# doing-science-to-stuff/ndt

Hardware: AMD Instinct MI355X
Metric: Mray/s (primary+shadow+reflect) at 1920x1080 (higher is better)
Workload: dtype f64

## Files before the change

ndt_amd/csrc/ndt_api.hip:

```cpp
#include "ndt_ctx.hpp"
#include <ctype.h>


static thread_local char g_err[512] = "";
int ndt_impl::fail(int code, const char *fmt, ...)
{
    va_list ap;
    va_start(ap, fmt);
    vsnprintf(g_err, sizeof(g_err), fmt, ap);
    va_end(ap);
    return code;
}

extern "C" const char *ndt_hip_last_error(void) { return g_err; }
extern "C" int ndt_hip_abi_version(void) { return NDT_HIP_ABI_VERSION; }

extern "C" int32_t ndt_hip_shard_rows(int32_t height, int32_t row_begin, int32_t row_step)
{
    if (row_step < 1 || row_begin < 0 || row_begin >= height) return 0;
    return (height - row_begin + row_step - 1) / row_step;
}

static const NdtKernelTable *table_for(int dims)
{
    switch (dims) {
    case 3: return ndt_kernel_table_3();
    case 4: return ndt_kernel_table_4();
    case 5: return ndt_kernel_table_5();
    case 6: return ndt_kernel_table_6();
    case 7: return ndt_kernel_table_7();
    case 8: return ndt_kernel_table_8();
    case 9: return ndt_kernel_table_9();
    case 10: return ndt_kernel_table_10();
    case 11: return ndt_kernel_table_11();
    case 12: return ndt_kernel_table_12();
    default: return nullptr;
    }
}

extern "C" int ndt_hip_create(int device, ndt_hip_ctx **out)
{
    if (!out) return fail(NDT_E_INVALID, "ndt_hip_create: out is NULL");
    *out = nullptr;
    int count = 0;
    hipError_t e = hipGetDeviceCount(&count);
    if (e != hipSuccess || count <= 0)
        return fail(NDT_E_DEVICE, "no HIP device available (%s); libndt_hip has no CPU path",
                    e == hipSuccess ? "device count is 0" : hipGetErrorString(e));
    if (device < 0 || device >= count) return fail(NDT_E_INVALID, "device %d out of range (have %d)", device, count);
    HIP_TRY(hipSetDevice(device));
    hipDeviceProp_t prop;
    HIP_TRY(hipGetDeviceProperties(&prop, device));
    if (strncmp(prop.gcnArchName, "gfx950", 6) != 0)
        return fail(NDT_E_DEVICE, "device %d is %s; this library carries gfx950 code objects only", device, prop.gcnArchName);
    ndt_hip_ctx *ctx = new ndt_hip_ctx();
    ctx->device = device;
    {
        static const char *const names[] = { "hybrid_level", "stream_below", "stream_below_list", "hull_box", "face_box", "face_tree", "face_groups", "item_sets", "gate_prepass", "gate_prepass_below", "item_boxes", "leaf_history", "leaf_scan", "leaf_scan_group", "multi_path", "sample_seed", "stream_fused", "fuse_primaries", "shade_pair", "light_window", "debug_levels",
                                             "exit_probe", "shade_probe", "stream_probe", "test_small_pool" };
        const char *pl = getenv("NDT_HIP_PIPELINE");
        if (pl) (void)ndt_hip_set_option(ctx, "pipeline", !strcmp(pl, "levels") ? 1 : !strcmp(pl, "stream") ? 2 : !strcmp(pl, "hybrid") ? 3 : 0);
        for (const char *nm : names) {
            char env[64] = "NDT_HIP_";
            size_t k = strlen(env);
            for (const char *q = nm; *q && k + 1 < sizeof(env); ++q) env[k++] = (char)toupper((unsigned char)*q);
            env[k] = 0;
            const char *v = getenv(env);
            if (v && *v) (void)ndt_hip_set_option(ctx, nm, !strcmp(nm, "shade_probe") ? atoll(v) + 1 : atoll(v));
        }
        if (getenv("NDT_HIP_NO_HULL_BOX")) ctx->hull_box = false;
        if (getenv("NDT_HIP_NO_FACE_BOX")) ctx->face_box = false;
        if (getenv("NDT_HIP_NO_SHADE_PAIR") && atoi(getenv("NDT_HIP_NO_SHADE_PAIR"))) ctx->shade_pair = false;
    }
    e = hipStreamCreateWithFlags(&ctx->stream, hipStreamNonBlocking);
    if (e != hipSuccess) {
        delete ctx;
        return fail(NDT_E_DEVICE, "hipStreamCreate: %s", hipGetErrorString(e));
    }
    e = hipHostMalloc((void **)&ctx->h_counters, 128 * sizeof(int), hipHostMallocDefault);
    if (e == hipSuccess) e = hipHostMalloc((void **)&ctx->h_levels, (NDT_MAX_LEVELS + 1) * sizeof(LevelRange), hipHostMallocDefault);
    if (e == hipSuccess) e = hipHostMalloc((void **)&ctx->h_mail, (NDT_MAX_LEVELS + 2) * sizeof(LevelRange), hipHostMallocMapped | hipHostMallocCoherent);
    if (e == hipSuccess) e = hipHostMalloc((void **)&ctx->h_mail_tag, (NDT_MAX_LEVELS + 2) * sizeof(unsigned long long), hipHostMallocMapped | hipHostMallocCoherent);
    if (e == hipSuccess) e = hipHostGetDevicePointer((void **)&ctx->d_mail, ctx->h_mail, 0);
    if (e == hipSuccess) e = hipHostGetDevicePointer((void **)&ctx->d_mail_tag, ctx->h_mail_tag, 0);
    if (e == hipSuccess) memset(ctx->h_mail_tag, 0, (NDT_MAX_LEVELS + 2) * sizeof(unsigned long long));
    if (e == hipSuccess) e = hipHostMalloc((void **)&ctx->h_done, 16 * sizeof(unsigned long long), hipHostMallocMapped | hipHostMallocCoherent);
    if (e == hipSuccess) e = hipHostGetDevicePointer((void **)&ctx->d_done, ctx->h_done, 0);
    if (e == hipSuccess) memset(ctx->h_done, 0, 16 * sizeof(unsigned long long));
    if (e != hipSuccess) {
        (void)hipStreamDestroy(ctx->stream);
        delete ctx;
        return fail(NDT_E_DEVICE, "hipHostMalloc: %s", hipGetErrorString(e));
    }
    *out = ctx;
    return NDT_OK;
}

extern "C" int ndt_hip_destroy(ndt_hip_ctx *ctx)
{
    if (!ctx) return NDT_OK;
    worker_stop(ctx);
    (void)hipSetDevice(ctx->device);
    (void)hipStreamSynchronize(ctx->stream);
    free_workspace(ctx);
    free_stage(ctx);
    free_async(ctx);
    if (ctx->d_shard) (void)hipFree(ctx->d_shard);
    if (ctx->d_image) (void)hipFree(ctx->d_image);
    for (auto &slot : ctx->pool)
        if (slot.first) (void)hipFree(slot.first);
    for (auto &slot : ctx->pool2)
        if (slot.first) (void)hipFree(slot.first);
    if (ctx->d_blob) (void)hipFree(ctx->d_blob);
    if (ctx->d_out) (void)hipFree(ctx->d_out);
    if (ctx->d_fit) (void)hipFree(ctx->d_fit);
    free_kd(ctx);
    free_png(ctx);
    free_jpeg(ctx);
    free_depth(ctx);
    free_ssaa(ctx);
    if (ctx->d_eyes) (void)hipFree(ctx->d_eyes);
    if (ctx->h_counters) (void)hipHostFree(ctx->h_counters);
    if (ctx->h_levels) (void)hipHostFree(ctx->h_levels);
    if (ctx->h_mail) (void)hipHostFree(ctx->h_mail);
    if (ctx->h_mail_tag) (void)hipHostFree(ctx->h_mail_tag);
    if (ctx->h_done) (void)hipHostFree(ctx->h_done);
    for (hipEvent_t ev : ctx->ev_pool) (void)hipEventDestroy(ev);
    (void)hipStreamDestroy(ctx->stream);
    delete ctx;
    return NDT_OK;
}

extern "C" int ndt_hip_set_option(ndt_hip_ctx *ctx, const char *name, int64_t value)
{
    if (!ctx || !name) return fail(NDT_E_INVALID, "NULL argument");
    const bool on = value != 0;
    if (!strcmp(name, "pipeline")) {
        if (value < 0 || value > 3) return fail(NDT_E_INVALID, "pipeline %lld", (long long)value);
        ctx->pipeline = (int)value;
    } else if (!strcmp(name, "hybrid_level")) ctx->hybrid_level = (int)value;
    else if (!strcmp(name, "stream_below")) ctx->stream_below = value;
    else if (!strcmp(name, "stream_below_list")) ctx->stream_below_list = value;
    else if (!strcmp(name, "hull_box")) ctx->hull_box = on;
    else if (!strcmp(name, "face_box")) ctx->face_box = on;
    else if (!strcmp(name, "face_tree")) ctx->face_tree = on;
    else if (!strcmp(name, "face_groups")) ctx->face_groups = on;
    else if (!strcmp(name, "item_sets")) ctx->item_sets = on;
    else if (!strcmp(name, "item_boxes")) ctx->item_boxes = on;
    else if (!strcmp(name, "gate_prepass_below")) ctx->gate_prepass_below = value;
    else if (!strcmp(name, "gate_prepass")) ctx->gate_prepass = value < 0 ? 0 : value > 2 ? 2 : (int)value;
    else if (!strcmp(name, "sample_seed")) ctx->sample_seed = value;
    else if (!strcmp(name, "leaf_scan")) ctx->leaf_scan = on;
    else if (!strcmp(name, "leaf_scan_group")) ctx->leaf_scan_group = value < 1 ? 1 : value > 64 ? 64 : (int)value;
    else if (!strcmp(name, "leaf_history")) ctx->leaf_history = value < 0 ? 0 : value > 4 ? 4 : (int)value;
    else if (!strcmp(name, "multi_path")) {
        if (value < 0 || value > 2) return fail(NDT_E_INVALID, "multi_path %lld", (long long)value);
        ctx->multi_path = (int)value;
    } else if (!strcmp(name, "stream_fused")) ctx->stream_fused = on;
    else if (!strcmp(name, "fuse_primaries")) ctx->fuse_primaries = value < 0 ? -1 : on ? 1 : 0;
    else if (!strcmp(name, "shade_pair")) ctx->shade_pair = on;
    else if (!strcmp(name, "light_window")) {
        if (value < 0 || value > 64) return fail(NDT_E_INVALID, "light_window %lld (0 auto, 1 .. 64)", (long long)value);
        ctx->light_window = (int)value;
        if (ctx->have_scene) light_windows(ctx);
    }
    else if (!strcmp(name, "debug_levels")) ctx->debug_levels = on;
    else if (!strcmp(name, "exit_probe")) ctx->exit_probe = on;
    else if (!strcmp(name, "shade_probe")) ctx->shade_probe = (int)value - 1;
    else if (!strcmp(name, "stream_probe")) ctx->stream_probe = on;
    else if (!strcmp(name, "test_small_pool")) ctx->test_small_pool = on;
    else return fail(NDT_E_INVALID, "unknown option '%s'", name);
    return NDT_OK;
}

extern "C" void *ndt_hip_stream(ndt_hip_ctx *ctx) { return ctx ? (void *)ctx->stream : nullptr; }
extern "C" int ndt_hip_synchronize(ndt_hip_ctx *ctx)
{
    if (!ctx) return fail(NDT_E_INVALID, "ctx is NULL");
    HIP_TRY(hipSetDevice(ctx->device));
    HIP_TRY(hipStreamSynchronize(ctx->stream));
    return NDT_OK;
}

extern "C" int ndt_hip_upload_scene(ndt_hip_ctx *ctx, const ndt_flat_scene *fs)
{
    if (!ctx || !fs) return fail(NDT_E_INVALID, "NULL argument");
    if (fs->abi_version != NDT_HIP_ABI_VERSION) return fail(NDT_E_INVALID, "scene ABI %d, library ABI %d", fs->abi_version, NDT_HIP_ABI_VERSION);
    if (fs->dims < NDT_MIN_DIMS || fs->dims > NDT_MAX_DIMS)
        return fail(NDT_E_UNSUPPORTED, "%d dimensions: kernels are built for %d..%d", fs->dims, NDT_MIN_DIMS, NDT_MAX_DIMS);
    if (fs->cam_type < 0 || fs->cam_type > 2) return fail(NDT_E_UNSUPPORTED, "camera type %d", fs->cam_type);
    if (fs->cam_type != 0 && (fs->cam_local_x_off < 0 || fs->cam_local_y_off < 0 || fs->cam_local_z_off < 0))
        return fail(NDT_E_INVALID, "VR / panorama cameras need the local axes (camera.h:69-71) in the flat scene");
    if (fs->n_lights < 0 || fs->n_lights > NDT_MAX_LIGHTS) return fail(NDT_E_UNSUPPORTED, "%d lights (max %d)", fs->n_lights, NDT_MAX_LIGHTS);
    if (fs->n_objects < 0 || fs->n_items < 0 || fs->n_items > fs->n_objects) return fail(NDT_E_INVALID, "object counts");
    if (fs->n_kd_nodes < 0 || fs->n_inf < 0 || fs->n_leaf_refs < 0) return fail(NDT_E_INVALID, "kd-tree counts");
    if (fs->n_objects > 0 && !fs->objects) return fail(NDT_E_INVALID, "objects is NULL");
    if (fs->n_lights > 0 && !fs->lights) return fail(NDT_E_INVALID, "lights is NULL");
    if (!fs->vecs) return fail(NDT_E_INVALID, "vecs is NULL");
    HIP_TRY(hipSetDevice(ctx->device));
    ctx->have_scene = false;
    int rc = build_blob(ctx, fs);
    if (rc) return rc;
    ctx->dims = fs->dims;
    ctx->kt = table_for(fs->dims);
    if (!ctx->kt) return fail(NDT_E_UNSUPPORTED, "no kernels for %d dimensions", fs->dims);
    HIP_TRY(hipStreamSynchronize(ctx->stream));
    if (ctx->d_blob_words < ctx->blob.size()) {
        if (ctx->d_blob) HIP_TRY(hipFree(ctx->d_blob));
        ctx->d_blob = nullptr;
        HIP_TRY(hipMalloc((void **)&ctx->d_blob, ctx->blob.size() * sizeof(double)));
        ctx->d_blob_words = ctx->blob.size();
    }
    HIP_TRY(hipMemcpyAsync(ctx->d_blob, ctx->blob.data(), ctx->blob.size() * sizeof(double), hipMemcpyHostToDevice, ctx->stream));
    HIP_TRY(hipStreamSynchronize(ctx->stream));
    ctx->aperture_radius = fs->cam_aperture_radius;
    ctx->have_scene = true;
    if (ctx->debug_levels)
        fprintf(stderr, "ndt_hip: scene blob: %d-D, %d items / %d objects, %d kd nodes of depth %d; %d words staged by the trace kernels (%d KB), %d in all; tier %d, %d mask word(s)\n",
                ctx->dims, ctx->sd.n_items, ctx->sd.n_objects, ctx->sd.n_kd_nodes, ctx->sd.kd_depth, ctx->sd.trace_words, ctx->sd.trace_words / 128,
                ctx->sd.total_words, ctx->tier, ctx->sd.mask_words);
    return NDT_OK;
}

__global__ void k_quantize(const double *rgba, unsigned char *out, long long n_values)
{
    const long long i = (long long)blockIdx.x * blockDim.x + threadIdx.x;
    if (i >= n_values) return;
    const double d = rgba[i];
    double m = (1.0 < d) ? 1.0 : d;
    m = (0.0 > m) ? 0.0 : m;
    out[i] = (unsigned char)(sqrt(m) * 255);
}

extern "C" int ndt_hip_quantize_device(ndt_hip_ctx *ctx, const void *d_rgba, void *d_rgba8, int64_t n_pixels)
{
    if (!ctx || !d_rgba || !d_rgba8 || n_pixels < 0) return fail(NDT_E_INVALID, "bad argument");
    HIP_TRY(hipSetDevice(ctx->device));
    const long long n = n_pixels * 4;
    if (n == 0) return NDT_OK;
// ... 81 lines not shown
```

ndt_amd/csrc/ndt_ctx.hpp:

```cpp
#pragma once
#include <hip/hip_runtime.h>
#include <hip/hip_ext.h>
#include <math.h>
#include <stdarg.h>
#include <stdio.h>
#include <stdlib.h>
#include <string.h>
#include <time.h>
#include <functional>
#include <string>
#include <vector>

#include "../../include/ndt_hip.h"
#include "ndt_kernels.hpp"

namespace ndt_impl {

struct CtxWorker;

int fail(int code, const char *fmt, ...) __attribute__((format(printf, 2, 3)));

}
using namespace ndt_impl;

// ... 20 lines not shown
           info_bytes = 0;
    void *h_info = nullptr;
};

struct JpegState {
    void *d_rgba8 = nullptr, *d_coef = nullptr, *d_slots = nullptr, *d_meta = nullptr, *d_offsets = nullptr, *d_file = nullptr, *d_info = nullptr;
    size_t rgba8_bytes = 0, coef_bytes = 0, slots_bytes = 0, meta_bytes = 0, offsets_bytes = 0, file_bytes = 0, info_bytes = 0;
    void *h_info = nullptr;
};

struct DepthState {
    void *d_records = nullptr;
    void *d_rgba8 = nullptr, *d_depth8 = nullptr;
    size_t records_bytes = 0, rgba8_bytes = 0, depth8_bytes = 0;
    void *h_result = nullptr;
    int launches = 0;
    double finish_ms = 0.0;
};

struct SsaaState {
    void *d_pass = nullptr;
    void *d_acc = nullptr;
    void *d_rgba8 = nullptr, *d_depth8 = nullptr;
    size_t pass_bytes = 0, acc_bytes = 0, rgba8_bytes = 0, depth8_bytes = 0;
    hipEvent_t ev[16] = {};
    int launches = 0;
    int factor = 0;
    double fold_ms = 0.0;
};

struct ndt_hip_ctx {
    int device = 0;
    hipStream_t stream = nullptr;
    const NdtKernelTable *kt = nullptr;
    int dims = 0;
    bool have_scene = false;
    double aperture_radius = 0.0;
    int cam_type = 0;
    bool have_eyes = false, have_local_axes = false;
    bool has_area_lights = false;
    SceneDesc sd{};
    std::vector<double> blob;
    double *d_blob = nullptr;
    size_t d_blob_words = 0;
    int tier = 0;
    int n_shadow_lights = 0;
    struct LightWindow {
        int first, count;
        int n_seg;
        unsigned long long ambient_bits;
    };
    int light_window = 0;
    std::vector<int> light_types;
    std::vector<LightWindow> windows;
    Workspace ws{};
    std::vector<void *> ws_allocs;
    std::vector<void *> sa_allocs;
    std::vector<std::pair<void *, size_t>> pool;
    std::vector<std::pair<void *, size_t>> pool2;
    long long ws_dims = 0;
    long long ws_slab_words = 0;
    int ws_nseg = 0;
    int pipeline = 0;
    int hybrid_level = 2;
    long long stream_below = 1000000;
    long long stream_below_list = 30000;
    StreamArgs sa{};
    bool stream_probe = false, exit_probe = false, debug_levels = false, test_small_pool = false;
    bool hull_box = true, face_box = true, shade_pair = true;
    bool face_tree = true;
    bool face_groups = true;
    int fuse_primaries = -1;
    bool stream_fused = true;
    bool item_sets = true;
    int gate_prepass = 2;
    long long gate_prepass_below = 400000;
    bool item_boxes = true;
    int leaf_scan_group = 64;
    bool leaf_scan = true;
    int leaf_history = 4;
    int shade_probe = -1;
    long long sa_cap = 0, sa_sh_cap = 0;
    int sa_nseg = 0;
    void *d_eyes = nullptr;
    size_t d_eyes_bytes = 0;
    void *d_fit = nullptr;
    size_t d_fit_bytes = 0;
    int fit_launches = 0;
    KdState kd;
    PngState png;
    JpegState jpeg;
    DepthState depth;
    SsaaState ssaa;
    void *d_out = nullptr;
    size_t d_out_bytes = 0;
    void *d_shard = nullptr;
    size_t d_shard_bytes = 0;
    void *d_image = nullptr;
    size_t d_image_bytes = 0;
    void *d_rgba8[2] = { nullptr, nullptr };
    size_t d_rgba8_bytes[2] = { 0, 0 };
    hipStream_t copy_stream = nullptr;
// ... 7 lines not shown
    long long sample_seed = 0;
    int multi_path = 0;
    int multi_path_taken = 0;
    ndt_impl::CtxWorker *worker = nullptr;
    int *h_counters = nullptr;
    LevelRange *h_levels = nullptr;
    LevelRange *h_mail = nullptr;
    unsigned long long *h_mail_tag = nullptr;
    LevelRange *d_mail = nullptr;
    unsigned long long *d_mail_tag = nullptr;
    unsigned long long frame_tag = 0;
    unsigned long long *h_done = nullptr;
    unsigned long long *d_done = nullptr;
    std::vector<hipEvent_t> ev_pool;
};

namespace ndt_impl {

struct HullFaces {
    std::vector<double> rows;
    std::vector<unsigned long long> possible;
    int n_faces = 0;
};
bool hcube_hull_box(const ndt_flat_scene *fs, const ndt_flat_object &o, int n, std::vector<double> &rows, HullFaces *faces = nullptr);
void hcube_face_tree(const HullFaces &hf, int n, std::vector<double> &rows, std::vector<int> &level_off, int &top);
void hcube_face_groups(const HullFaces &hf, const std::vector<double> &hull_rows, int n, std::vector<double> &clusters, std::vector<int> &table,
                       std::vector<int> &face_set, std::vector<int> &members);
bool scene_item_boxes(const ndt_flat_scene *fs, int n, std::vector<double> &frame, std::vector<double> &rows, std::vector<char> &has);
int build_blob(ndt_hip_ctx *ctx, const ndt_flat_scene *fs);
void light_windows(ndt_hip_ctx *ctx);
SceneDesc window_desc(const ndt_hip_ctx *ctx, const SceneDesc &sd, int k);

void free_workspace(ndt_hip_ctx *ctx);
int ensure_workspace(ndt_hip_ctx *ctx, long long cap, long long sh_cap);
int render_pass(ndt_hip_ctx *ctx, RenderGeom rg, bool prof, void *d_rgba, ndt_render_stats &st, void *d_depth = nullptr);
void launch_fill_black(hipStream_t s, double *rgba, long long n_pixels);
void add_stats(ndt_render_stats &acc, const ndt_render_stats &st);

void print_stream_probe(const unsigned int *wave_log, float kernel_ms);
void print_shade_probe(const unsigned int *shade_log, int shade_probe, long long finish_waves);
void print_exit_probe(const unsigned int *exit_log, int launches);
void print_phase_timing(const unsigned long long *dbg);

void worker_stop(ndt_hip_ctx *ctx);
void free_stage(ndt_hip_ctx *ctx);
void free_async(ndt_hip_ctx *ctx);

int fit_spheres_device(ndt_hip_ctx *ctx, int dims, long long n_lists, const int64_t *first, const double *points, const double *point_radius,
                       double *centers, double *radii);

int build_kdtree_device(ndt_hip_ctx *ctx, int dims, int n_items, const double *lower, const double *upper, const unsigned char *finite);
void free_kd(ndt_hip_ctx *ctx);

void free_png(ndt_hip_ctx *ctx);

void free_jpeg(ndt_hip_ctx *ctx);

void free_depth(ndt_hip_ctx *ctx);

void free_ssaa(ndt_hip_ctx *ctx);

int render_antialiased(ndt_hip_ctx *ctx, const ndt_render_params *p, void *d_rgba, ndt_render_stats &total, void *d_depth = nullptr);
void launch_anaglyph(hipStream_t s, const double *left, const double *right, double *out, long long n_pixels);
int render_sampled(ndt_hip_ctx *ctx, const ndt_render_params *p, void *d_rgba, ndt_render_stats &total, void *d_depth = nullptr);
struct SampledList {
    const double *d_pos;
// ... 85 lines not shown
```

ndt_amd/csrc/ndt_frame.hip:

```cpp
#include "ndt_ctx.hpp"
#include "ndt_finish.hpp"
#include <stddef.h>

static void free_stream_args(ndt_hip_ctx *ctx)
{
    for (void *p : ctx->sa_allocs) (void)hipFree(p);
    ctx->sa_allocs.clear();
    memset(&ctx->sa, 0, sizeof(ctx->sa));
    ctx->sa_cap = ctx->sa_sh_cap = 0;
    ctx->sa_nseg = 0;
}

void ndt_impl::free_workspace(ndt_hip_ctx *ctx)
{
    for (void *p : ctx->ws_allocs) (void)hipFree(p);
    ctx->ws_allocs.clear();
    free_stream_args(ctx);
    memset(&ctx->ws, 0, sizeof(ctx->ws));
    ctx->ws_slab_words = 0;
    ctx->ws_dims = 0;
    ctx->ws_nseg = 0;
}


template <typename T> static int ws_alloc(ndt_hip_ctx *ctx, T **p, size_t count, bool stream_args = false)
{
    void *q = nullptr;
    hipError_t e = hipMalloc(&q, (count > 0 ? count : 1) * sizeof(T));
    if (e != hipSuccess) {
        (void)hipGetLastError();
        return fail(NDT_E_NOMEM, "hipMalloc of %zu bytes: %s", count * sizeof(T), hipGetErrorString(e));
    }
    (stream_args ? ctx->sa_allocs : ctx->ws_allocs).push_back(q);
    *p = (T *)q;
    return NDT_OK;
}

int ndt_impl::ensure_workspace(ndt_hip_ctx *ctx, long long cap, long long sh_cap)
{
    Workspace &ws = ctx->ws;
    const bool need_slab = ctx->tier == 1;
    const long long slab_lanes = 2048LL * NDT_TRACE_BLOCK;
    const long long slab_words = need_slab ? slab_lanes * ctx->sd.mask_words : 0;
    if (ws.cap >= cap && ws.sh_cap >= sh_cap && ctx->ws_dims == ctx->dims && ctx->ws_slab_words >= slab_words &&
        ctx->ws_nseg >= ctx->n_shadow_lights)
        return NDT_OK;
    if (cap < ws.cap) cap = ws.cap;
    if (sh_cap < ws.sh_cap) sh_cap = ws.sh_cap;
    cap = (cap + 63) & ~63LL;
    sh_cap = (sh_cap + 63) & ~63LL;
    HIP_TRY(hipStreamSynchronize(ctx->stream));
    free_workspace(ctx);
    const int n = ctx->dims;
    int rc;
    auto give_up = [&](int code) {
        free_workspace(ctx);
        return code;
    };
    ws.cap = cap;
    ws.sh_cap = sh_cap;
    if ((rc = ws_alloc(ctx, &ws.ray_o, (size_t)n * cap))) return give_up(rc);
    if ((rc = ws_alloc(ctx, &ws.ray_v, (size_t)n * cap))) return give_up(rc);
    if ((rc = ws_alloc(ctx, &ws.frac, (size_t)cap))) return give_up(rc);
    if ((rc = ws_alloc(ctx, &ws.depth, (size_t)cap))) return give_up(rc);
    if ((rc = ws_alloc(ctx, &ws.rng_key, (size_t)cap))) return give_up(rc);
    if ((rc = ws_alloc(ctx, &ws.depth_left, (size_t)cap))) return give_up(rc);
    if ((rc = ws_alloc(ctx, &ws.hit_obj, (size_t)cap))) return give_up(rc);
    if ((rc = ws_alloc(ctx, &ws.hit_prim, (size_t)cap))) return give_up(rc);
    if ((rc = ws_alloc(ctx, &ws.hit_p, (size_t)n * cap))) return give_up(rc);
    if ((rc = ws_alloc(ctx, &ws.hit_n, (size_t)n * cap))) return give_up(rc);
    if ((rc = ws_alloc(ctx, &ws.clr, (size_t)3 * cap))) return give_up(rc);
    if ((rc = ws_alloc(ctx, &ws.child_refl, (size_t)cap))) return give_up(rc);
    if ((rc = ws_alloc(ctx, &ws.child_refr, (size_t)cap))) return give_up(rc);
    if ((rc = ws_alloc(ctx, &ws.sh_idx, (size_t)cap * (ctx->n_shadow_lights > 0 ? ctx->n_shadow_lights : 1)))) return give_up(rc);
    if ((rc = ws_alloc(ctx, &ws.sh_mask, (size_t)cap))) return give_up(rc);
    if ((rc = ws_alloc(ctx, &ws.count, (size_t)cap))) return give_up(rc);
    if ((rc = ws_alloc(ctx, &ws.so, (size_t)n * sh_cap))) return give_up(rc);
    if ((rc = ws_alloc(ctx, &ws.sv, (size_t)n * sh_cap))) return give_up(rc);
    if ((rc = ws_alloc(ctx, &ws.slim, (size_t)sh_cap))) return give_up(rc);
    if ((rc = ws_alloc(ctx, &ws.sobj, (size_t)sh_cap))) return give_up(rc);
    if ((rc = ws_alloc(ctx, &ws.sprim, (size_t)sh_cap))) return give_up(rc);
    if ((rc = ws_alloc(ctx, &ws.counters, NDT_CNT_ALLOC))) return give_up(rc);
    if ((rc = ws_alloc(ctx, &ws.ref_rays, 64 * 8))) return give_up(rc);
    if ((rc = ws_alloc(ctx, &ws.dbg, 160))) return give_up(rc);
    if ((rc = ws_alloc(ctx, &ws.exit_log, (size_t)NDT_EXIT_LOG_LAUNCHES * NDT_EXIT_LOG_WORDS))) return give_up(rc);
    if (ctx->shade_probe >= 0 && (rc = ws_alloc(ctx, &ws.shade_log, (size_t)2 * NDT_SHADE_LOG_WAVES))) return give_up(rc);
    if ((rc = ws_alloc(ctx, &ws.levels, NDT_MAX_LEVELS + 1))) return give_up(rc);
    ws.mask_slab_lanes = slab_lanes;
    if (need_slab) {
        if ((rc = ws_alloc(ctx, &ws.mask_slab, (size_t)slab_words))) return give_up(rc);
    }
    ctx->ws_slab_words = slab_words;
    ctx->ws_dims = ctx->dims;
    ctx->ws_nseg = ctx->n_shadow_lights > 0 ? ctx->n_shadow_lights : 1;
    return NDT_OK;
}

static int ensure_stream_args(ndt_hip_ctx *ctx)
{
    const Workspace &ws = ctx->ws;
    const int n_seg = ctx->n_shadow_lights > 0 ? ctx->n_shadow_lights : 1;
    if (ctx->sa.ctl && ctx->sa_cap == ws.cap && ctx->sa_sh_cap == ws.sh_cap && ctx->sa_nseg == n_seg) return NDT_OK;
    if (!ctx->sa_allocs.empty()) {
        HIP_TRY(hipStreamSynchronize(ctx->stream));
        free_stream_args(ctx);
    }
    StreamArgs &sa = ctx->sa;
    const long long margin = NDT_STREAM_LOG_WAVES;
    const long long node_batches = ws.cap / 64 + margin;
    const long long seg_cap = (ws.sh_cap / n_seg) & ~63LL;
    const long long sh_batches = (long long)n_seg * (seg_cap / 64) + margin;
    int rc;
    if ((rc = ws_alloc(ctx, &sa.ctl, 1, true))) return rc;
    if ((rc = ws_alloc(ctx, &sa.node_fill, (size_t)node_batches, true))) return rc;
    if ((rc = ws_alloc(ctx, &sa.sh_pending, (size_t)node_batches, true))) return rc;
    if ((rc = ws_alloc(ctx, &sa.sh_fill, (size_t)sh_batches, true))) return rc;
    if ((rc = ws_alloc(ctx, &sa.sec_ring, (size_t)NDT_PRIM_SHARDS * node_batches, true))) return rc;
    if ((rc = ws_alloc(ctx, &sa.sh_ring, (size_t)sh_batches, true))) return rc;
    if ((rc = ws_alloc(ctx, &sa.fin_ring, (size_t)node_batches, true))) return rc;
    if ((rc = ws_alloc(ctx, &sa.parent, (size_t)ws.cap, true))) return rc;
    if ((rc = ws_alloc(ctx, &sa.pend, (size_t)ws.cap, true))) return rc;
    if ((rc = ws_alloc(ctx, &sa.sowner, (size_t)n_seg * seg_cap, true))) return rc;
    if (ctx->stream_probe && (rc = ws_alloc(ctx, &sa.wave_log, (size_t)24 * NDT_STREAM_LOG_WAVES, true))) return rc;
    sa.n_seg = n_seg;
    sa.seg_cap = (int)seg_cap;
    sa.node_batches = (int)node_batches;
    ctx->sa_cap = ws.cap;
    ctx->sa_sh_cap = ws.sh_cap;
    ctx->sa_nseg = n_seg;
    return NDT_OK;
}


__global__ void k_frame_init(Workspace ws, int n_primary, LevelRange level0, int queue_ints)
{
    const int i = blockIdx.x * blockDim.x + threadIdx.x, stride = gridDim.x * blockDim.x;
    for (int k = i; k < queue_ints; k += stride) ws.counters[NDT_CNT_QUEUE + k] = 0;
// ... 285 lines not shown
        st.rays_secondary = (long long)ctx->h_done[6];
        st.rays_shadow = (long long)ctx->h_done[3];
        st.rays_ref_equiv = (long long)ctx->h_done[5];
        st.levels = (int)ctx->h_done[4];
        st.trace_launches = 1;
        st.node_capacity = ws.cap;
        if (prof) {
            float km = 0, fm = 0;
            HIP_TRY(hipEventElapsedTime(&km, ev_k0, ev_k1));
            HIP_TRY(hipEventElapsedTime(&fm, ev_begin, ev_end));
            st.trace_ms = km;
            st.frame_ms = fm;
            if (sa.wave_log) print_stream_probe(sa.wave_log, km);
        }
        return NDT_OK;
    }
    return fail(NDT_E_NOMEM, "ray-tree workspace kept overflowing");
}

struct FrameInFlight {
    ndt_hip_ctx *ctx;
    const RenderGeom &rg;
    const SceneDesc &sd_pass;
    const bool prof;
    const bool hybrid;
    void *d_rgba, *d_depth;
    hipStream_t s;
    const NdtKernelTable *kt;
    Workspace ws;
    const int n_levels;
    const int hand;
    const int n_win;
    const bool windowed;
    std::vector<SceneDesc> sd_win;
    int win_emits = 0;
    unsigned long long tag = 0;
    int slots = 0, queue_slot = 0;
    int launches = 0;
    size_t ev_n = 0;
    hipEvent_t ev_begin = nullptr, ev_end = nullptr, ev_k0 = nullptr, ev_k1 = nullptr;
    std::vector<std::pair<hipEvent_t, hipEvent_t>> trace_ev;
    std::vector<std::string> trace_dbg;
    int shade_launch = 0;
    long long shade_probe_finish_waves = 0;
    int n_run;
    std::vector<long long> level_nodes;
    int pending_finish = -1;
    long long pending_upper = 0;
    bool resolve_with_finish = false;
    StreamArgs sa{};
    bool streamed = false;

    FrameInFlight(ndt_hip_ctx *c, const RenderGeom &g, const SceneDesc &sd, bool p, bool hyb, void *rgba, void *depth)
        : ctx(c), rg(g), sd_pass(sd), prof(p), hybrid(hyb), d_rgba(rgba), d_depth(depth), s(c->stream), kt(c->kt), ws(c->ws),
          n_levels(g.max_depth > 1 ? g.max_depth : 1), hand(hyb ? c->hybrid_level : n_levels + 1), n_win((int)c->windows.size()),
          windowed(n_win > 1), n_run(n_levels)
    {
        ws.mail = ctx->d_mail;
        ws.mail_tag = ctx->d_mail_tag;
        for (int k = 0; windowed && k < n_win; ++k) sd_win.push_back(window_desc(ctx, sd_pass, k));
    }

    int render(long long &cap, long long &sh_cap, ndt_render_stats &st);
    int frame_init(long long &sh_cap);
    int traced(TraceJob &tj, const std::string &what, const SceneDesc *sd_job = nullptr);
    Workspace shade_ws(long long finish_nodes);
    int trace_primaries();
    void light_and_shade(int b, long long upper);
    int trace_bounce(int b, long long upper);
    int trace_windows(int b, long long upper);
    void light_last();
    int hand_off(long long &cap);
    void resolve();
    int close();
    int report(long long &cap, long long &sh_cap, ndt_render_stats &st);
    hipError_t print_debug(int levels_used);
};

int FrameInFlight::render(long long &cap, long long &sh_cap, ndt_render_stats &st)
{
    int rc;
    if ((rc = frame_init(sh_cap))) return rc;
    if ((rc = trace_primaries())) return rc;
    long long upper = rg.n_primary;
    for (int b = 0; b < n_levels && b < hand; ++b) {
        if ((windowed ? b + 2 : queue_slot + 1) > NDT_QUEUE_SLOTS || b + 1 > NDT_MAX_LEVELS)
            return fail(NDT_E_UNSUPPORTED, "more than %d bounces", NDT_QUEUE_SLOTS - 1);
        if (b > 0) {
            if ((rc = wait_for_tag(ctx, &ctx->h_mail_tag[b], tag, "bounce %d was never published", b))) return rc;
            upper = ctx->h_mail[b].count;
            if (upper <= 0) {
                n_run = b;
                break;
            }
        }
        level_nodes.push_back(upper);
        light_and_shade(b, upper);
        if ((rc = trace_bounce(b, upper))) return rc;
        if (windowed && (rc = trace_windows(b, upper))) return rc;
        pending_finish = b;
        pending_upper = upper;
    }
    light_last();
    if (hybrid && n_run >= hand && hand < n_levels && (rc = hand_off(cap))) return rc;
    resolve();
    launch_finish_pixels(ctx, sd_pass, ws, rg, d_rgba, d_depth, n_run >= 1 ? 1 : 0);
    if ((rc = close())) return rc;
    return report(cap, sh_cap, st);
}

int FrameInFlight::frame_init(long long &sh_cap)
{
    if (prof) {
        ev_begin = get_event(ctx, ev_n++);
        ev_end = get_event(ctx, ev_n++);
    }
    if (prof && ctx->exit_probe)
        HIP_TRY(hipMemsetAsync(ws.exit_log, 0, (size_t)NDT_EXIT_LOG_LAUNCHES * NDT_EXIT_LOG_WORDS * sizeof(unsigned int), s));
    tag = ++ctx->frame_tag;
    LevelRange level0;
    level0.begin = 0;
    level0.count = rg.n_primary;
    level0.seg_stride = (rg.n_primary + 63) & ~63LL;
    level0.n_shadow = 0;
    if ((long long)ctx->n_shadow_lights * level0.seg_stride > ws.sh_cap) {
        sh_cap = (long long)ctx->n_shadow_lights * level0.seg_stride;
        return PASS_AGAIN;
    }
    const long long want_slots = (long long)n_levels * (windowed ? n_win : 1) + 2;
    slots = want_slots > NDT_QUEUE_SLOTS ? NDT_QUEUE_SLOTS : (int)want_slots;
    launch_stamped(k_frame_init, dim3(8), dim3(256), s, ev_begin, nullptr, ws, rg.n_primary, level0, slots * NDT_QUEUE_INTS);
    if (windowed) HIP_TRY(hipMemsetAsync(ws.counters + NDT_CNT_WIN, 0, (NDT_CNT_ALLOC - NDT_CNT_WIN) * sizeof(int), s));
    return NDT_OK;
}

int FrameInFlight::traced(TraceJob &tj, const std::string &what, const SceneDesc *sd_job)
{
    tj.queue = ws.counters + NDT_CNT_QUEUE + (queue_slot % NDT_QUEUE_SLOTS) * NDT_QUEUE_INTS;
    if (queue_slot++ >= slots) HIP_TRY(hipMemsetAsync(tj.queue, 0, NDT_QUEUE_INTS * sizeof(int), s));
    const SceneDesc &sdj = sd_job ? *sd_job : sd_pass;
    tj.exit_log = (ctx->exit_probe && prof && launches < NDT_EXIT_LOG_LAUNCHES) ? ws.exit_log + (size_t)launches * NDT_EXIT_LOG_WORDS : nullptr;
    hipEvent_t a = nullptr, b2 = nullptr;
    if (prof) {
        a = get_event(ctx, ev_n++);
        b2 = get_event(ctx, ev_n++);
        trace_ev.push_back({ a, b2 });
        trace_dbg.push_back(what);
    }
    kt->trace(s, ctx->d_blob, sdj, ws, tj, ctx->tier, ctx->sd.mask_words, a, b2);
    ++launches;
    return NDT_OK;
}

Workspace FrameInFlight::shade_ws(long long finish_nodes)
{
    Workspace w = ws;
    if (shade_launch++ != ctx->shade_probe || !prof) {
        w.shade_log = nullptr;
    } else {
        shade_probe_finish_waves = (finish_nodes + 255) / 256 * 4;
        (void)hipMemsetAsync(w.shade_log, 0, (size_t)2 * NDT_SHADE_LOG_WAVES * sizeof(unsigned int), s);
    }
    return w;
}

static void job_closest(TraceJob &tj, const Workspace &ws)
{
    tj.dense.o = ws.ray_o; tj.dense.v = ws.ray_v; tj.dense.stride = ws.cap; tj.dense.lim = nullptr;
    tj.dense.valid = ws.depth_left; tj.dense.out_obj = ws.hit_obj; tj.dense.out_prim = ws.hit_prim;
    tj.begin = 0;
}

static void job_shadow(TraceJob &tj, const Workspace &ws, const SceneDesc &sd_pass, int b, long long upper, int n_seg, const int *seg_count)
{
    tj.n_seg = n_seg;
    tj.seg.o = ws.so; tj.seg.v = ws.sv; tj.seg.stride = ws.sh_cap; tj.seg.lim = ws.slim; tj.seg.valid = nullptr;
    tj.seg_light_origins = sd_pass.light_origins;
    tj.seg.out_obj = ws.sobj; tj.seg.out_prim = ws.sprim;
    tj.seg_count = seg_count;
    tj.seg_stride = (upper + 63) & ~63LL;
    tj.levels = ws.levels;
    tj.seg_level = b;
}

int FrameInFlight::trace_primaries()
{
    const bool fuse_primaries = (ctx->fuse_primaries < 0 ? ctx->dims >= 4 : ctx->fuse_primaries != 0) && ctx->cam_type == 0;
    if (!fuse_primaries) kt->primary(s, ctx->d_blob, sd_pass, ws, rg);
    TraceJob tj{};
    job_closest(tj, ws);
    tj.count = rg.n_primary;
    tj.publish_level = -1;
    if (fuse_primaries) {
        tj.make_primaries = 1;
        tj.rg = rg;
    }
    return traced(tj, "primaries + closest 0");
}

void FrameInFlight::light_and_shade(int b, long long upper)
{
    if (windowed) {
        if (pending_finish >= 0)
            kt->shade_last(s, ctx->d_blob, sd_win[n_win - 1], shade_ws(pending_upper), rg, pending_finish, pending_upper, 0, ctx->windows[n_win - 1].first);
        kt->shade_emit(s, ctx->d_blob, sd_win[0], shade_ws(0), rg, b, upper);
    } else if (pending_finish >= 0 && ctx->shade_pair) {
        kt->shade_pair(s, ctx->d_blob, sd_pass, shade_ws(pending_upper), rg, pending_finish, pending_upper, upper);
    } else {
        if (pending_finish >= 0) kt->shade_finish(s, ctx->d_blob, sd_pass, shade_ws(pending_upper), rg, pending_finish, pending_upper, 0);
        kt->shade_emit(s, ctx->d_blob, sd_pass, shade_ws(0), rg, b, upper);
    }
    pending_finish = -1;
}

int FrameInFlight::trace_bounce(int b, long long upper)
{
    long long next_upper = 2 * upper;
    if (next_upper > ws.cap) next_upper = ws.cap;
    const bool last = b + 1 == hand;
    TraceJob tj{};
    job_shadow(tj, ws, sd_pass, b, upper, windowed ? ctx->windows[0].n_seg : ctx->n_shadow_lights, NDT_SEG_COUNTERS(ws, b));
    job_closest(tj, ws);
    tj.count = next_upper;
    tj.dense_level = last ? -1 : b + 1;
    tj.publish_level = b;
    tj.publish_tag = tag;
    return traced(tj, "shadow " + std::to_string(b) + (last ? "" : " + closest " + std::to_string(b + 1)), windowed ? &sd_win[0] : nullptr);
}

int FrameInFlight::trace_windows(int b, long long upper)
{
    for (int k = 1; k < n_win; ++k) {
        const ndt_hip_ctx::LightWindow &w = ctx->windows[k];
        int *bank = ws.counters + NDT_CNT_WIN + 64 * (win_emits & 1);
        int *next_bank = ws.counters + NDT_CNT_WIN + 64 * ((win_emits + 1) & 1);
        ++win_emits;
        kt->shade_window(s, ctx->d_blob, sd_win[k - 1], sd_win[k], shade_ws(upper), rg, b, upper, ctx->windows[k - 1].first, w.first, bank, next_bank,
                         w.n_seg, k > 1 ? 1 : 0);
        if (w.n_seg == 0) continue;
        TraceJob tj{};
        job_shadow(tj, ws, sd_pass, b, upper, w.n_seg, bank);
        tj.count = 0;
        tj.dense_level = -1;
        tj.publish_level = -1;
        int rc = traced(tj, "shadow " + std::to_string(b) + " window " + std::to_string(k), &sd_win[k]);
        if (rc) return rc;
    }
    return NDT_OK;
}

void FrameInFlight::light_last()
{
    if (pending_finish < 0) return;
    resolve_with_finish = !hybrid && pending_finish >= 1 && pending_finish == n_run - 1;
    if (windowed)
        kt->shade_last(s, ctx->d_blob, sd_win[n_win - 1], shade_ws(pending_upper), rg, pending_finish, pending_upper, resolve_with_finish ? 1 : 0,
                       ctx->windows[n_win - 1].first);
    else
        kt->shade_finish(s, ctx->d_blob, sd_pass, shade_ws(pending_upper), rg, pending_finish, pending_upper, resolve_with_finish ? 1 : 0);
}

int FrameInFlight::hand_off(long long &cap)
{
    int rc;
    if ((rc = wait_for_tag(ctx, &ctx->h_mail_tag[hand], tag, "bounce %d was never published", hand))) return rc;
    const LevelRange roots = ctx->h_mail[hand];
    if (roots.count > 0) {
        if ((rc = stream_roots(ctx, prof, roots.begin, roots.count, 0, sa))) return rc;
        if ((long long)sa.root_begin + sa.n_primary > ws.cap) {
            cap *= 2;
            return PASS_AGAIN;
        }
        launch_stream_init(ctx, ws, sa, 0, nullptr);
        if (prof) {
            ev_k0 = get_event(ctx, ev_n++);
            ev_k1 = get_event(ctx, ev_n++);
            trace_ev.push_back({ ev_k0, ev_k1 });
            trace_dbg.push_back("frame kernel, bounces " + std::to_string(hand) + " ..");
        }
        kt->frame_stream(s, ctx->d_blob, sd_pass, ws, rg, sa, ctx->tier, ctx->sd.mask_words, ev_k0, ev_k1);
        ++launches;
        streamed = true;
    }
    n_run = hand;
    return NDT_OK;
}

void FrameInFlight::resolve()
{
    for (int b = n_run; b-- > 1;) {
        if (resolve_with_finish && b == n_run - 1) continue;
        long long blocks = (level_nodes[b] + 255) / 256;
// ... 121 lines not shown
```

profiles/timeline.py:

```python
#!/usr/bin/env python3
import csv
import sys
rows = list(csv.DictReader(open(sys.argv[1])))
ks = [(r['Kernel_Name'].split('(')[0][-34:], int(r['Start_Timestamp']), int(r['End_Timestamp'])) for r in rows]
ks.sort(key=lambda x: x[1])
idx = [i for i, k in enumerate(ks) if 'k_frame_init' in k[0]]
i0, i1 = idx[-2], idx[-1]
t0 = ks[i0][1]
prev_end = t0
for k in ks[i0:i1]:
    print("%-36s start %8.1f us  dur %7.1f us  gap %6.1f us" % (k[0], (k[1] - t0) / 1e3, (k[2] - k[1]) / 1e3, (k[1] - prev_end) / 1e3))
    prev_end = k[2]
print("frame span %.1f us" % ((ks[i1][1] - t0) / 1e3))
```

Baseline: 3950.

## Run shade-finish on a low-priority light stream beside later bounces

Adds a second, lowest-priority HIP stream and, for non-windowed non-hybrid frames, moves each bounce's shade_finish onto it. It runs two levels behind the main trace/emit chain, synchronised by events and triple-banked shadow answer buffers (sobj/sprim now 3x sh_cap). The goal is to overlap lighting work with subsequent tracing kernels instead of serialising them, and it gives up the fused shade_pair path. The costs are extra events, cross-stream waits, triple the shadow-output memory, and possible contention with the main stream.

```diff
diff --git a/ndt_amd/csrc/ndt_api.hip b/ndt_amd/csrc/ndt_api.hip
--- a/ndt_amd/csrc/ndt_api.hip
+++ b/ndt_amd/csrc/ndt_api.hip
@@ -56,7 +56,7 @@
     ndt_hip_ctx *ctx = new ndt_hip_ctx();
     ctx->device = device;
     {
-        static const char *const names[] = { "hybrid_level", "stream_below", "stream_below_list", "hull_box", "face_box", "face_tree", "face_groups", "item_sets", "gate_prepass", "gate_prepass_below", "item_boxes", "leaf_history", "leaf_scan", "leaf_scan_group", "multi_path", "sample_seed", "stream_fused", "fuse_primaries", "shade_pair", "light_window", "debug_levels",
+        static const char *const names[] = { "hybrid_level", "stream_below", "stream_below_list", "hull_box", "face_box", "face_tree", "face_groups", "item_sets", "gate_prepass", "gate_prepass_below", "item_boxes", "leaf_history", "leaf_scan", "leaf_scan_group", "multi_path", "sample_seed", "stream_fused", "fuse_primaries", "shade_pair", "light_overlap", "light_window", "debug_levels",
                                              "exit_probe", "shade_probe", "stream_probe", "test_small_pool" };
         const char *pl = getenv("NDT_HIP_PIPELINE");
         if (pl) (void)ndt_hip_set_option(ctx, "pipeline", !strcmp(pl, "levels") ? 1 : !strcmp(pl, "stream") ? 2 : !strcmp(pl, "hybrid") ? 3 : 0);
@@ -73,6 +73,12 @@
         if (getenv("NDT_HIP_NO_SHADE_PAIR") && atoi(getenv("NDT_HIP_NO_SHADE_PAIR"))) ctx->shade_pair = false;
     }
     e = hipStreamCreateWithFlags(&ctx->stream, hipStreamNonBlocking);
+    if (e == hipSuccess) {
+        int least = 0, greatest = 0;
+        e = hipDeviceGetStreamPriorityRange(&least, &greatest);
+        if (e == hipSuccess) e = hipStreamCreateWithPriority(&ctx->light_stream, hipStreamNonBlocking, least);
+        if (e != hipSuccess) (void)hipStreamDestroy(ctx->stream);
+    }
     if (e != hipSuccess) {
         delete ctx;
         return fail(NDT_E_DEVICE, "hipStreamCreate: %s", hipGetErrorString(e));
@@ -88,6 +94,7 @@
     if (e == hipSuccess) e = hipHostGetDevicePointer((void **)&ctx->d_done, ctx->h_done, 0);
     if (e == hipSuccess) memset(ctx->h_done, 0, 16 * sizeof(unsigned long long));
     if (e != hipSuccess) {
+        (void)hipStreamDestroy(ctx->light_stream);
         (void)hipStreamDestroy(ctx->stream);
         delete ctx;
         return fail(NDT_E_DEVICE, "hipHostMalloc: %s", hipGetErrorString(e));
@@ -101,7 +108,7 @@
     if (!ctx) return NDT_OK;
     worker_stop(ctx);
     (void)hipSetDevice(ctx->device);
-    (void)hipStreamSynchronize(ctx->stream);
+    (void)sync_streams(ctx);
     free_workspace(ctx);
     free_stage(ctx);
     free_async(ctx);
@@ -126,6 +133,7 @@
     if (ctx->h_mail_tag) (void)hipHostFree(ctx->h_mail_tag);
     if (ctx->h_done) (void)hipHostFree(ctx->h_done);
     for (hipEvent_t ev : ctx->ev_pool) (void)hipEventDestroy(ev);
+    (void)hipStreamDestroy(ctx->light_stream);
     (void)hipStreamDestroy(ctx->stream);
     delete ctx;
     return NDT_OK;
@@ -159,6 +167,7 @@
     } else if (!strcmp(name, "stream_fused")) ctx->stream_fused = on;
     else if (!strcmp(name, "fuse_primaries")) ctx->fuse_primaries = value < 0 ? -1 : on ? 1 : 0;
     else if (!strcmp(name, "shade_pair")) ctx->shade_pair = on;
+    else if (!strcmp(name, "light_overlap")) ctx->light_overlap = on;
     else if (!strcmp(name, "light_window")) {
         if (value < 0 || value > 64) return fail(NDT_E_INVALID, "light_window %lld (0 auto, 1 .. 64)", (long long)value);
         ctx->light_window = (int)value;
@@ -204,7 +213,7 @@
     ctx->dims = fs->dims;
     ctx->kt = table_for(fs->dims);
     if (!ctx->kt) return fail(NDT_E_UNSUPPORTED, "no kernels for %d dimensions", fs->dims);
-    HIP_TRY(hipStreamSynchronize(ctx->stream));
+    HIP_TRY(sync_streams(ctx));
     if (ctx->d_blob_words < ctx->blob.size()) {
         if (ctx->d_blob) HIP_TRY(hipFree(ctx->d_blob));
         ctx->d_blob = nullptr;
diff --git a/ndt_amd/csrc/ndt_ctx.hpp b/ndt_amd/csrc/ndt_ctx.hpp
--- a/ndt_amd/csrc/ndt_ctx.hpp
+++ b/ndt_amd/csrc/ndt_ctx.hpp
@@ -76,6 +76,7 @@
 struct ndt_hip_ctx {
     int device = 0;
     hipStream_t stream = nullptr;
+    hipStream_t light_stream = nullptr;
     const NdtKernelTable *kt = nullptr;
     int dims = 0;
     bool have_scene = false;
@@ -112,6 +113,7 @@
     StreamArgs sa{};
     bool stream_probe = false, exit_probe = false, debug_levels = false, test_small_pool = false;
     bool hull_box = true, face_box = true, shade_pair = true;
+    bool light_overlap = true;
     bool face_tree = true;
     bool face_groups = true;
     int fuse_primaries = -1;
@@ -185,6 +187,7 @@
 SceneDesc window_desc(const ndt_hip_ctx *ctx, const SceneDesc &sd, int k);
 
 void free_workspace(ndt_hip_ctx *ctx);
+hipError_t sync_streams(ndt_hip_ctx *ctx);
 int ensure_workspace(ndt_hip_ctx *ctx, long long cap, long long sh_cap);
 int render_pass(ndt_hip_ctx *ctx, RenderGeom rg, bool prof, void *d_rgba, ndt_render_stats &st, void *d_depth = nullptr);
 void launch_fill_black(hipStream_t s, double *rgba, long long n_pixels);
diff --git a/ndt_amd/csrc/ndt_frame.hip b/ndt_amd/csrc/ndt_frame.hip
--- a/ndt_amd/csrc/ndt_frame.hip
+++ b/ndt_amd/csrc/ndt_frame.hip
@@ -9,6 +9,13 @@
     memset(&ctx->sa, 0, sizeof(ctx->sa));
     ctx->sa_cap = ctx->sa_sh_cap = 0;
     ctx->sa_nseg = 0;
+}
+
+hipError_t ndt_impl::sync_streams(ndt_hip_ctx *ctx)
+{
+    const hipError_t e = hipStreamSynchronize(ctx->stream);
+    if (e != hipSuccess || !ctx->light_stream) return e;
+    return hipStreamSynchronize(ctx->light_stream);
 }
 
 void ndt_impl::free_workspace(ndt_hip_ctx *ctx)
@@ -49,7 +56,7 @@
     if (sh_cap < ws.sh_cap) sh_cap = ws.sh_cap;
     cap = (cap + 63) & ~63LL;
     sh_cap = (sh_cap + 63) & ~63LL;
-    HIP_TRY(hipStreamSynchronize(ctx->stream));
+    HIP_TRY(sync_streams(ctx));
     free_workspace(ctx);
     const int n = ctx->dims;
     int rc;
@@ -78,8 +85,8 @@
     if ((rc = ws_alloc(ctx, &ws.so, (size_t)n * sh_cap))) return give_up(rc);
     if ((rc = ws_alloc(ctx, &ws.sv, (size_t)n * sh_cap))) return give_up(rc);
     if ((rc = ws_alloc(ctx, &ws.slim, (size_t)sh_cap))) return give_up(rc);
-    if ((rc = ws_alloc(ctx, &ws.sobj, (size_t)sh_cap))) return give_up(rc);
-    if ((rc = ws_alloc(ctx, &ws.sprim, (size_t)sh_cap))) return give_up(rc);
+    if ((rc = ws_alloc(ctx, &ws.sobj, (size_t)3 * sh_cap))) return give_up(rc);
+    if ((rc = ws_alloc(ctx, &ws.sprim, (size_t)3 * sh_cap))) return give_up(rc);
     if ((rc = ws_alloc(ctx, &ws.counters, NDT_CNT_ALLOC))) return give_up(rc);
     if ((rc = ws_alloc(ctx, &ws.ref_rays, 64 * 8))) return give_up(rc);
     if ((rc = ws_alloc(ctx, &ws.dbg, 160))) return give_up(rc);
@@ -102,7 +109,7 @@
     const int n_seg = ctx->n_shadow_lights > 0 ? ctx->n_shadow_lights : 1;
     if (ctx->sa.ctl && ctx->sa_cap == ws.cap && ctx->sa_sh_cap == ws.sh_cap && ctx->sa_nseg == n_seg) return NDT_OK;
     if (!ctx->sa_allocs.empty()) {
-        HIP_TRY(hipStreamSynchronize(ctx->stream));
+        HIP_TRY(sync_streams(ctx));
         free_stream_args(ctx);
     }
     StreamArgs &sa = ctx->sa;
@@ -454,6 +461,11 @@
     const int hand;
     const int n_win;
     const bool windowed;
+    const bool overlap;
+    hipStream_t ls;
+    hipEvent_t ev_lit[3] = { nullptr, nullptr, nullptr };
+    int light_next = 0;
+    hipEvent_t light_tail = nullptr;
     std::vector<SceneDesc> sd_win;
     int win_emits = 0;
     unsigned long long tag = 0;
@@ -476,7 +488,7 @@
     FrameInFlight(ndt_hip_ctx *c, const RenderGeom &g, const SceneDesc &sd, bool p, bool hyb, void *rgba, void *depth)
         : ctx(c), rg(g), sd_pass(sd), prof(p), hybrid(hyb), d_rgba(rgba), d_depth(depth), s(c->stream), kt(c->kt), ws(c->ws),
           n_levels(g.max_depth > 1 ? g.max_depth : 1), hand(hyb ? c->hybrid_level : n_levels + 1), n_win((int)c->windows.size()),
-          windowed(n_win > 1), n_run(n_levels)
+          windowed(n_win > 1), overlap(c->light_overlap && !windowed && !hyb), ls(c->light_stream), n_run(n_levels)
     {
         ws.mail = ctx->d_mail;
         ws.mail_tag = ctx->d_mail_tag;
@@ -484,11 +496,15 @@
     }
 
     int render(long long &cap, long long &sh_cap, ndt_render_stats &st);
+    int render_frame(long long &cap, long long &sh_cap, ndt_render_stats &st);
     int frame_init(long long &sh_cap);
     int traced(TraceJob &tj, const std::string &what, const SceneDesc *sd_job = nullptr);
-    Workspace shade_ws(long long finish_nodes);
+    int answer_bank(int b) const { return overlap ? b % 3 : 0; }
+    Workspace shade_ws(long long finish_nodes, int b, hipStream_t on);
     int trace_primaries();
     void light_and_shade(int b, long long upper);
+    int light_beside(int b);
+    hipError_t join_light();
     int trace_bounce(int b, long long upper);
     int trace_windows(int b, long long upper);
     void light_last();
@@ -500,6 +516,31 @@
 };
 
 int FrameInFlight::render(long long &cap, long long &sh_cap, ndt_render_stats &st)
+{
+    const int rc = render_frame(cap, sh_cap, st);
+    const hipError_t e = join_light();
+    if (rc == NDT_OK && e != hipSuccess) return fail(NDT_E_DEVICE, "joining the light stream: %s", hipGetErrorString(e));
+    return rc;
+}
+
+hipError_t FrameInFlight::join_light()
+{
+    if (!light_tail) return hipSuccess;
+    const hipError_t e = hipStreamWaitEvent(s, light_tail, 0);
+    light_tail = nullptr;
+    return e;
+}
+
+int FrameInFlight::light_beside(int b)
+{
+    kt->shade_finish(ls, ctx->d_blob, sd_pass, shade_ws(level_nodes[b], b, ls), rg, b, level_nodes[b], 0);
+    HIP_TRY(hipEventRecord(ev_lit[b % 3], ls));
+    light_tail = ev_lit[b % 3];
+    light_next = b + 1;
+    return NDT_OK;
+}
+
+int FrameInFlight::render_frame(long long &cap, long long &sh_cap, ndt_render_stats &st)
 {
     int rc;
     if ((rc = frame_init(sh_cap))) return rc;
@@ -511,6 +552,7 @@
         if (b > 0) {
             if ((rc = wait_for_tag(ctx, &ctx->h_mail_tag[b], tag, "bounce %d was never published", b))) return rc;
             upper = ctx->h_mail[b].count;
+            if (overlap && b >= 2 && (rc = light_beside(b - 2))) return rc;
             if (upper <= 0) {
                 n_run = b;
                 break;
@@ -524,7 +566,12 @@
         pending_upper = upper;
     }
     light_last();
+    if (overlap && n_run >= 2 && light_next == n_run - 2) {
+        if ((rc = wait_for_tag(ctx, &ctx->h_mail_tag[n_run], tag, "bounce %d was never published", n_run))) return rc;
+        if ((rc = light_beside(n_run - 2))) return rc;
+    }
     if (hybrid && n_run >= hand && hand < n_levels && (rc = hand_off(cap))) return rc;
+    HIP_TRY(join_light());
     resolve();
     launch_finish_pixels(ctx, sd_pass, ws, rg, d_rgba, d_depth, n_run >= 1 ? 1 : 0);
     if ((rc = close())) return rc;
@@ -537,6 +584,8 @@
         ev_begin = get_event(ctx, ev_n++);
         ev_end = get_event(ctx, ev_n++);
     }
+    for (int p = 0; overlap && p < 3; ++p)
+        if (!(ev_lit[p] = get_event(ctx, ev_n++))) return fail(NDT_E_DEVICE, "hipEventCreate failed");
     if (prof && ctx->exit_probe)
         HIP_TRY(hipMemsetAsync(ws.exit_log, 0, (size_t)NDT_EXIT_LOG_LAUNCHES * NDT_EXIT_LOG_WORDS * sizeof(unsigned int), s));
     tag = ++ctx->frame_tag;
@@ -574,14 +623,16 @@
     return NDT_OK;
 }
 
-Workspace FrameInFlight::shade_ws(long long finish_nodes)
+Workspace FrameInFlight::shade_ws(long long finish_nodes, int b, hipStream_t on)
 {
     Workspace w = ws;
+    w.sobj += answer_bank(b) * ws.sh_cap;
+    w.sprim += answer_bank(b) * ws.sh_cap;
     if (shade_launch++ != ctx->shade_probe || !prof) {
         w.shade_log = nullptr;
     } else {
         shade_probe_finish_waves = (finish_nodes + 255) / 256 * 4;
-        (void)hipMemsetAsync(w.shade_log, 0, (size_t)2 * NDT_SHADE_LOG_WAVES * sizeof(unsigned int), s);
+        (void)hipMemsetAsync(w.shade_log, 0, (size_t)2 * NDT_SHADE_LOG_WAVES * sizeof(unsigned int), on);
     }
     return w;
 }
@@ -593,12 +644,13 @@
     tj.begin = 0;
 }
 
-static void job_shadow(TraceJob &tj, const Workspace &ws, const SceneDesc &sd_pass, int b, long long upper, int n_seg, const int *seg_count)
+static void job_shadow(TraceJob &tj, const Workspace &ws, const SceneDesc &sd_pass, int b, long long upper, int n_seg, const int *seg_count,
+                       int bank = 0)
 {
     tj.n_seg = n_seg;
     tj.seg.o = ws.so; tj.seg.v = ws.sv; tj.seg.stride = ws.sh_cap; tj.seg.lim = ws.slim; tj.seg.valid = nullptr;
     tj.seg_light_origins = sd_pass.light_origins;
-    tj.seg.out_obj = ws.sobj; tj.seg.out_prim = ws.sprim;
+    tj.seg.out_obj = ws.sobj + bank * ws.sh_cap; tj.seg.out_prim = ws.sprim + bank * ws.sh_cap;
     tj.seg_count = seg_count;
     tj.seg_stride = (upper + 63) & ~63LL;
     tj.levels = ws.levels;
@@ -624,13 +676,17 @@
 {
     if (windowed) {
         if (pending_finish >= 0)
-            kt->shade_last(s, ctx->d_blob, sd_win[n_win - 1], shade_ws(pending_upper), rg, pending_finish, pending_upper, 0, ctx->windows[n_win - 1].first);
-        kt->shade_emit(s, ctx->d_blob, sd_win[0], shade_ws(0), rg, b, upper);
+            kt->shade_last(s, ctx->d_blob, sd_win[n_win - 1], shade_ws(pending_upper, pending_finish, s), rg, pending_finish, pending_upper, 0,
+                           ctx->windows[n_win - 1].first);
+        kt->shade_emit(s, ctx->d_blob, sd_win[0], shade_ws(0, b, s), rg, b, upper);
+    } else if (overlap) {
+        kt->shade_emit(s, ctx->d_blob, sd_pass, shade_ws(0, b, s), rg, b, upper);
     } else if (pending_finish >= 0 && ctx->shade_pair) {
-        kt->shade_pair(s, ctx->d_blob, sd_pass, shade_ws(pending_upper), rg, pending_finish, pending_upper, upper);
+        kt->shade_pair(s, ctx->d_blob, sd_pass, shade_ws(pending_upper, pending_finish, s), rg, pending_finish, pending_upper, upper);
     } else {
-        if (pending_finish >= 0) kt->shade_finish(s, ctx->d_blob, sd_pass, shade_ws(pending_upper), rg, pending_finish, pending_upper, 0);
-        kt->shade_emit(s, ctx->d_blob, sd_pass, shade_ws(0), rg, b, upper);
+        if (pending_finish >= 0)
+            kt->shade_finish(s, ctx->d_blob, sd_pass, shade_ws(pending_upper, pending_finish, s), rg, pending_finish, pending_upper, 0);
+        kt->shade_emit(s, ctx->d_blob, sd_pass, shade_ws(0, b, s), rg, b, upper);
     }
     pending_finish = -1;
 }
@@ -641,12 +697,13 @@
     if (next_upper > ws.cap) next_upper = ws.cap;
     const bool last = b + 1 == hand;
     TraceJob tj{};
-    job_shadow(tj, ws, sd_pass, b, upper, windowed ? ctx->windows[0].n_seg : ctx->n_shadow_lights, NDT_SEG_COUNTERS(ws, b));
+    job_shadow(tj, ws, sd_pass, b, upper, windowed ? ctx->windows[0].n_seg : ctx->n_shadow_lights, NDT_SEG_COUNTERS(ws, b), answer_bank(b));
     job_closest(tj, ws);
     tj.count = next_upper;
     tj.dense_level = last ? -1 : b + 1;
     tj.publish_level = b;
     tj.publish_tag = tag;
+    if (overlap && b >= 3) HIP_TRY(hipStreamWaitEvent(s, ev_lit[b % 3], 0));
     return traced(tj, "shadow " + std::to_string(b) + (last ? "" : " + closest " + std::to_string(b + 1)), windowed ? &sd_win[0] : nullptr);
 }
 
@@ -657,7 +714,7 @@
         int *bank = ws.counters + NDT_CNT_WIN + 64 * (win_emits & 1);
         int *next_bank = ws.counters + NDT_CNT_WIN + 64 * ((win_emits + 1) & 1);
         ++win_emits;
-        kt->shade_window(s, ctx->d_blob, sd_win[k - 1], sd_win[k], shade_ws(upper), rg, b, upper, ctx->windows[k - 1].first, w.first, bank, next_bank,
+        kt->shade_window(s, ctx->d_blob, sd_win[k - 1], sd_win[k], shade_ws(upper, b, s), rg, b, upper, ctx->windows[k - 1].first, w.first, bank, next_bank,
                          w.n_seg, k > 1 ? 1 : 0);
         if (w.n_seg == 0) continue;
         TraceJob tj{};
@@ -676,10 +733,11 @@
     if (pending_finish < 0) return;
     resolve_with_finish = !hybrid && pending_finish >= 1 && pending_finish == n_run - 1;
     if (windowed)
-        kt->shade_last(s, ctx->d_blob, sd_win[n_win - 1], shade_ws(pending_upper), rg, pending_finish, pending_upper, resolve_with_finish ? 1 : 0,
-                       ctx->windows[n_win - 1].first);
+        kt->shade_last(s, ctx->d_blob, sd_win[n_win - 1], shade_ws(pending_upper, pending_finish, s), rg, pending_finish, pending_upper,
+                       resolve_with_finish ? 1 : 0, ctx->windows[n_win - 1].first);
     else
-        kt->shade_finish(s, ctx->d_blob, sd_pass, shade_ws(pending_upper), rg, pending_finish, pending_upper, resolve_with_finish ? 1 : 0);
+        kt->shade_finish(s, ctx->d_blob, sd_pass, shade_ws(pending_upper, pending_finish, s), rg, pending_finish, pending_upper,
+                         resolve_with_finish ? 1 : 0);
 }
 
 int FrameInFlight::hand_off(long long &cap)
diff --git a/profiles/timeline.py b/profiles/timeline.py
--- a/profiles/timeline.py
+++ b/profiles/timeline.py
@@ -1,14 +1,40 @@
-#!/usr/bin/env python3
+import collections
 import csv
+import statistics
 import sys
-rows = list(csv.DictReader(open(sys.argv[1])))
-ks = [(r['Kernel_Name'].split('(')[0][-34:], int(r['Start_Timestamp']), int(r['End_Timestamp'])) for r in rows]
-ks.sort(key=lambda x: x[1])
-idx = [i for i, k in enumerate(ks) if 'k_frame_init' in k[0]]
-i0, i1 = idx[-2], idx[-1]
-t0 = ks[i0][1]
-prev_end = t0
-for k in ks[i0:i1]:
-    print("%-36s start %8.1f us  dur %7.1f us  gap %6.1f us" % (k[0], (k[1] - t0) / 1e3, (k[2] - k[1]) / 1e3, (k[1] - prev_end) / 1e3))
-    prev_end = k[2]
-print("frame span %.1f us" % ((ks[i1][1] - t0) / 1e3))
+
+rows = sorted(csv.DictReader(open(sys.argv[1])), key=lambda r: int(r["Start_Timestamp"]))
+frames, cur = [], None
+for r in rows:
+    name = r["Kernel_Name"].split("(")[0]
+    if name.endswith("k_frame_init"):
+        cur = []
+        frames.append(cur)
+    if cur is not None:
+        cur.append((name[-40:], int(r["Start_Timestamp"]), int(r["End_Timestamp"]), r.get("Queue_Id", "?")))
+        if name.endswith("k_frame_done"):
+            cur = None
+frames = [f for f in frames if f[-1][0].endswith("k_frame_done")]
+if not frames:
+    sys.exit("no complete frame in the trace")
+span = lambda f: max(k[2] for k in f) - f[0][1]
+mid = sorted(frames, key=span)[len(frames) // 2]
+t0, last_end = mid[0][1], mid[0][1]
+for name, a, b, q in mid:
+    print("%-40s queue %-3s start %7.1f us  dur %6.1f us  gap %7.1f us" % (name, q, (a - t0) / 1e3, (b - a) / 1e3, (a - last_end) / 1e3))
+    last_end = max(last_end, b)
+print("frame span %.1f us (median of %d frames: %.1f us)" % (span(mid) / 1e3, len(frames), statistics.median(span(f) for f in frames) / 1e3))
+by_place = collections.defaultdict(list)
+for f in frames:
+    seen = collections.Counter()
+    for name, a, b, q in f:
+        by_place[(name, seen[name])].append((b - a) / 1e3)
+        seen[name] += 1
+order = []
+for name, a, b, q in mid:
+    order.append(name)
+seen = collections.Counter()
+for name in order:
+    v = by_place[(name, seen[name])]
+    print("  %-40s #%d  n=%4d median %7.1f us  min %7.1f" % (name, seen[name], len(v), statistics.median(v), min(v)))
+    seen[name] += 1
```

Result: faster. 4344, median of 6 (+10.0%).
